# ktncktnc/diffusion-forcing-transformer

Measured on AMD Instinct MI355X. Metric: denoised latent frames/sec, DFoT RE10K 8f & 200f rollout @1/2/4/8 GPU, higher is better.
Workload: dtype bf16

## Files before the change

### diffusion-forcing-transformer_amd/capi.py

```python
from __future__ import annotations

import ctypes as C
import os

_HERE = os.path.dirname(os.path.abspath(__file__))
LIB_PATH = os.environ.get("DFOT_LIB", os.path.join(_HERE, "libdfot_hip.so"))

OK, ERR_ARG, ERR_SHAPE, ERR_HIP, ERR_STATE, ERR_NAME = range(6)


class DfotError(RuntimeError):
    def __init__(self, code: int, message: str):
        super().__init__(f"libdfot_hip error {code}: {message}")
        self.code = code


class UViTConfig(C.Structure):
    _fields_ = [
        ("channels", C.c_int32 * 4), ("emb_channels", C.c_int32), ("num_updown_blocks", C.c_int32 * 3),
        ("num_mid_blocks", C.c_int32), ("num_heads", C.c_int32), ("in_channels", C.c_int32),
        ("resolution", C.c_int32), ("max_tokens", C.c_int32), ("cond_dim", C.c_int32), ("noise_dim", C.c_int32),
        ("rope_theta", C.c_float), ("eps", C.c_float),
    ]

# ... 23 lines not shown
ATTN_MAP_OFF, ATTN_MAP_FRAME, ATTN_MAP_FULL = -1, 0, 1


_P, _I, _L, _F = C.c_void_p, C.c_int, C.c_int64, C.c_float
_I32 = C.c_int32


class GemmDesc(C.Structure):
    _fields_ = [
        ("amode", _I32), ("epi", _I32), ("variant", _I32),
        ("A", _P), ("lda", _L), ("W", _P), ("ldw", _L),
        ("M", _I32), ("N", _I32), ("K", _I32), ("H", _I32), ("Wd", _I32), ("Cin", _I32),
        ("live", _P), ("bias", _P), ("bias_rows", _I32),
        ("out_f32", _P), ("out_bf16", _P), ("ldo", _L),
        ("resid", _P), ("resid_bf", _P),
        ("gate", _P), ("gate_index", _P), ("ldg", _L), ("gate_rows", _I32),
        ("act", _I32), ("pre_act", _P), ("raw", _P), ("ldraw", _L), ("tr_rows", _I32),
        ("gn_part", _P), ("gn_rows_per_bt", _I32), ("gn_cpg", _I32),
        ("out2", _P), ("ldo2", _L), ("split", _I32),
        ("q", _P), ("k", _P), ("v", _P),
        ("qw", _P), ("kw", _P), ("rope_cs", _P),
        ("heads", _I32), ("d", _I32), ("ntok", _I32), ("qscale", _F), ("dstride", _I32), ("eps", _F),
        ("ksplit", _I32), ("slice_stride", _L),
    ]


SIGNATURES = {
    "dfot_last_error": (C.c_char_p, []),
    "dfot_version": (_I, []),
    "dfot_uvit_create": (_I, [C.POINTER(UViTConfig), C.POINTER(_P)]),
    "dfot_uvit_destroy": (_I, [_P]),
    "dfot_uvit_num_params": (_I, [_P]),
    "dfot_uvit_param_name": (C.c_char_p, [_P, _I]),
    "dfot_uvit_param_shape": (_I, [_P, _I, C.POINTER(_L), C.POINTER(_I)]),
    "dfot_uvit_load_weight": (_I, [_P, C.c_char_p, _P, C.POINTER(_L), _I, _P]),
    "dfot_uvit_finalize": (_I, [_P, _P]),
    "dfot_uvit_reserve": (_I, [_P, _I]),
    "dfot_uvit_workspace_bytes": (C.c_size_t, [_P]),
    "dfot_uvit_set_option": (_I, [_P, C.c_char_p, _I]),
    "dfot_uvit_query": (_I, [_P, C.c_char_p, C.POINTER(C.c_double)]),
    "dfot_uvit_attn_timing": (_I, [_P, C.POINTER(C.c_double), C.POINTER(_L)]),
    "dfot_uvit_forward": (_I, [_P, _P, _P, _P, _P, _P, _I, _P]),
    "dfot_uvit_set_conditions": (_I, [_P, _P, _P, _I, _P]),
    "dfot_uvit_forward_cached": (_I, [_P, _P, _P, _P, _I, _P]),
    "dfot_uvit_forward_cached_live": (_I, [_P, _P, _P, _P, _I, _P, _P]),
    "dfot_uvit_forward_cached_masks": (_I, [_P, _P, _P, _P, _I, _P, _P, _P]),
    "dfot_uvit_read_tap": (_I, [_P, C.c_char_p, _P, C.c_size_t, _P]),
    "dfot_uvit3d_create": (_I, [C.POINTER(UViT3DConfig), C.POINTER(_P)]),
    "dfot_uvit3d_config_bytes": (_L, []),
    "dfot_uvit3d_forward": (_I, [_P, _P, _P, _P, _P, _P, _I, _P]),
    "dfot_uvit3d_forward_live": (_I, [_P, _P, _P, _P, _P, _P, _I, _P, _P]),
    "dfot_op_gn_film_silu": (_I, [_P, _P, _P, _P, _P, _P, _P, _P, _I, _I, _I, _I, _P]),
    "dfot_op_rms_film": (_I, [_P, _P, _P, _P, _P, _P, _L, _I, _I, _I, _F, _P]),
    "dfot_dit_create": (_I, [C.POINTER(DiTConfig), C.POINTER(_P)]),
    "dfot_dit_create_f": (_I, [C.POINTER(DiTConfigF), C.POINTER(_P)]),
    "dfot_dit_destroy": (_I, [_P]),
    "dfot_dit_num_params": (_I, [_P]),
    "dfot_dit_param_name": (C.c_char_p, [_P, _I]),
    "dfot_dit_param_shape": (_I, [_P, _I, C.POINTER(_L), C.POINTER(_I)]),
    "dfot_dit_load_weight": (_I, [_P, C.c_char_p, _P, C.POINTER(_L), _I, _P]),
    "dfot_dit_finalize": (_I, [_P, _P]),
    "dfot_dit_reserve": (_I, [_P, _I]),
    "dfot_dit_workspace_bytes": (C.c_size_t, [_P]),
    "dfot_dit_set_option": (_I, [_P, C.c_char_p, _I]),
    "dfot_dit_attn_timing": (_I, [_P, C.POINTER(C.c_double), C.POINTER(_L)]),
    "dfot_dit_forward": (_I, [_P, _P, _P, _P, _I, _I, _P]),
    "dfot_dit_forward_cond": (_I, [_P, _P, _P, _P, _P, _P, _P, _I, _I, _P]),
    "dfot_dit_forward_f": (_I, [_P, _P, _P, _P, _P, _P, _P, _I, _I, _P]),
    "dfot_dit_read_tap": (_I, [_P, C.c_char_p, _P, C.c_size_t, _P]),
    "dfot_dit_capture_attention": (_I, [_P, C.POINTER(_I32), _I, _I, C.c_size_t]),
    "dfot_dit_attention_map_shape": (_I, [_P, _I, C.POINTER(_L), C.POINTER(_I)]),
    "dfot_dit_read_attention_map": (_I, [_P, _I, _P, C.c_size_t, _P]),
    "dfot_dit_train_create": (_I, [C.POINTER(DiTConfig), C.POINTER(_P)]),
    "dfot_dit_train_create_f": (_I, [C.POINTER(DiTConfigF), C.POINTER(_P)]),
    "dfot_facmat_train_create": (_I, [C.POINTER(DiTConfigF), C.POINTER(_P)]),
    "dfot_facdit_train_create": (_I, [C.POINTER(DiTConfigF), C.POINTER(_P)]),
    "dfot_dit_train_destroy": (_I, [_P]),
    "dfot_dit_train_num_params": (_I, [_P]),
    "dfot_dit_train_param_name": (C.c_char_p, [_P, _I]),
    "dfot_dit_train_param_shape": (_I, [_P, _I, C.POINTER(_L), C.POINTER(_I)]),
    "dfot_dit_train_param_offset": (_L, [_P, _I]),
    "dfot_dit_train_total_numel": (_L, [_P]),
    "dfot_dit_train_workspace_bytes": (C.c_size_t, [_P]),
    "dfot_dit_train_attach": (_I, [_P, _P, _P]),
    "dfot_dit_train_reserve": (_I, [_P, _I]),
    "dfot_dit_train_sync_weights": (_I, [_P, _P]),
    "dfot_dit_train_forward": (_I, [_P, _P, _P, _P, _I, _I, _P]),
    "dfot_dit_train_forward_cond": (_I, [_P, _P, _P, _P, _P, _P, _P, _I, _I, _P]),
    "dfot_dit_train_load_buffer": (_I, [_P, C.c_char_p, _P, _L, _P]),
    "dfot_dit_train_forward_f": (_I, [_P, _P, _P, _P, _P, _P, _P, _I, _I, _P]),
    "dfot_dit_train_input_grad": (_I, [_P, _P, _P]),
    "dfot_dit_train_backward": (_I, [_P, _P, _P]),
    "dfot_vloss_grad": (_I, [_P] * 7 + [_I, _I, _L, _I, _P]),
    "dfot_sumsq": (_I, [_P, _L, _P, _P]),
    "dfot_adamw_step": (_I, [_P, _P, _P, _P, _L, _F, _F, _F, _F, _F, _I, _P, _F, _P, _F, _P]),
    "dfot_ray_encode": (_I, [_P, _P, _I, _I, _I, _P]),
    "dfot_ray_encode_normalized": (_I, [_P, _P, _I, _I, _I, _P]),
    "dfot_hg_prepare": (_I, [_P, _P, _P, _P, _P, _I, _I, _I, _L, _P]),
    "dfot_ddim_compose": (_I, [_P] * 11 + [_I, _I, _I, _L, _P]),
    "dfot_ddim_compose_tokw": (_I, [_P] * 11 + [_I, _I, _I, _L, _P]),
    "dfot_ddim_noise": (_I, [_P] * 5 + [_I, _I, _I, _L, _I, _P]),
    "dfot_vpred_loss": (_I, [_P] * 9 + [_I, _I, _L, _P]),
    "dfot_vpred_loss_scratch_floats": (_L, [_I, _I, _L]),
    "dfot_vspace_loss": (_I, [_P] * 9 + [_I, _I, _L, _P]),
    "dfot_op_gemm": (_I, [_P, _I, _P, _P, _P, _I, _I, _I, _I, _P]),
    "dfot_op_conv3x3": (_I, [_P, _P, _P, _P, _I, _I, _I, _I, _I, _I, _P]),
# ... 133 lines not shown
```

### diffusion-forcing-transformer_amd/csrc/kernels.h

```cpp
#pragma once
#include "common.h"

namespace dfot {

int launch_noise_emb(const float* k, const float* freqs, const float* phases, const float* w1, const float* b1,
                     const float* w2, const float* b2, float* hidden, float* out, int bt, int ndim, int e, hipStream_t s);
int launch_uvit3d_emb(const float* k, const float* freqs, const float* phases, const float* w1, const float* b1, const float* w2,
                      const float* b2, const float* cond, const uint8_t* cond_mask, const float* a_w1, const float* a_b1,
                      const float* a_w2, const float* a_b2, float* out, int bt, int ndim, int cdim, int e, int tokens, hipStream_t s);
int launch_embed_input(const float* x, const float* w, const float* b, float* out, int bt, int res, int cin, int c0,
                       hipStream_t s);
int launch_cond_repack(const float* cond, bf16* a, int bt, int res, int cdim, int kpad, hipStream_t s);
int launch_emb_pyramid(const bf16* emb0, bf16* emb1, bf16* emb2, bf16* emb3, int bt, int r0, int e, hipStream_t s);
int launch_project_output(const float* x0, const float* w, const float* b, float* out, int bt, int res, int c0, int cout,
                          hipStream_t s, const uint8_t* live = nullptr);
int launch_gn_partial_f32(const float* x, float* partial, int bt, int pixels, int c, hipStream_t s);
int launch_gn_partial_bf16(const bf16* x, float* partial, int bt, int pixels, int c, hipStream_t s);
int launch_gn_finalize(const float* partial, float* stats, int bt, int nblk, int pixels, int c, float eps, hipStream_t s);
int gn_partial_blocks(int pixels);
int launch_gn_apply_silu(const float* x, const float* stats, const float* gamma, const float* beta, bf16* out, int bt,
                         int pixels, int c, hipStream_t s, const uint8_t* live = nullptr);
struct FilmChunk {
  const bf16* w;
  const float* b;
  long out_off;
  int rows;
};
int launch_film_vec(const FilmChunk* table, int chunks, const float* nemb, float* sv, int bt, int e, hipStream_t s);
int launch_gn_film_silu(const bf16* h, const float* stats, const float* gamma, const float* beta, const bf16* fcache,
                        const float* sv, const uint8_t* cond_mask, bf16* out, int bt, int pixels, int c, int tokens,
                        hipStream_t s, const uint8_t* live = nullptr);
struct RmsPending {
  void* x;
  const float* bias;
  const float* s0;
  const float* s1;
  const float* s2;
};
int launch_rms_film(const float* x, const float* w, const bf16* fcache, const float* sv, const uint8_t* cond_mask, bf16* out,
                    long m, int c, int rows_per_bt, int tokens, float eps, hipStream_t s, const RmsPending* pend = nullptr);
int launch_rms_film_bf16(const bf16* x, const float* w, const bf16* fcache, const float* sv, const uint8_t* cond_mask, bf16* out,
                         long m, int c, int rows_per_bt, int tokens, float eps, hipStream_t s, const RmsPending* pend = nullptr);

int launch_pool2_bf16(const float* x, bf16* out, int bt, int h, int w, int c, hipStream_t s);
int launch_pool2_bf16_bf16in(const bf16* x, bf16* out, int bt, int h, int w, int c, hipStream_t s);
int launch_sub_bf16_bf16in(const bf16* a, const float* b, bf16* out, long n, hipStream_t s, const uint8_t* live = nullptr, long frame_elems = 0);
int launch_upsample_add_bf16(const float* t, const bf16* skip, bf16* out, int bt, int h, int w, int c, hipStream_t s, const uint8_t* live = nullptr);
int launch_gn_apply_silu_bf16in(const bf16* x, const float* stats, const float* gamma, const float* beta, bf16* out, int bt, int pixels, int c,
                                hipStream_t s, const uint8_t* live = nullptr);
int launch_embed_input_bf16(const float* x, const float* w, const float* b, bf16* out, int bt, int res, int cin, int c0, hipStream_t s);
int launch_project_output_bf16(const bf16* x0, const float* w, const float* b, float* out, int bt, int res, int c0, int cout, hipStream_t s,
                               const uint8_t* live = nullptr);
int launch_sub_bf16(const float* a, const float* b, bf16* out, long n, hipStream_t s, const uint8_t* live = nullptr, long frame_elems = 0);
int launch_upsample_add(const float* t, const float* skip, float* out, int bt, int h, int w, int c, hipStream_t s, const uint8_t* live = nullptr);
int launch_ray_encode(const float* poses, float* out, int b, int t, int res, int normalized, hipStream_t s);
int launch_hg_prepare(const float* x, const float* noise, const float* qa, const float* qb, float* x_in, int batch,
                      int nfe, int tokens, long f, hipStream_t s);
int launch_ddim_compose(const float* x, const float* x_in, const float* v, const float* sa, const float* s1,
                        const float* an, const float* cn, const float* keep, const float* weight, const uint8_t* gen,
                        float* x_next, int batch, int nfe, int tokens, long f, bool weight_per_token, hipStream_t s);
int launch_ddim_noise(const float* noise, const float* sigma, const float* weight, const uint8_t* gen, float* x_next, int batch, int nfe,
                      int tokens, long f, bool weight_per_token, hipStream_t s);
int vloss_chunks(long f);
int launch_vloss(const float* x, const float* noise, const float* v, const float* a, const float* sg, const float* w,
                 float* x_pred, float* partial, float* loss, int batch, int tokens, long f, bool vspace, hipStream_t s);
int launch_wgrad_nt(const bf16* a, long lda, const bf16* b, long ldb, float* out, int m, int n, long rows, int slices, hipStream_t s, int img_h = 0,
                    int img_w = 0, int sdy = 0, int sdx = 0, int all_taps = 0);
struct WgradPlan {
  int form, slices;
};
WgradPlan wgrad_plan(int m, int n, long rows, long max_slices);
int launch_wgrad_conv_taps(const bf16* dy, const bf16* x, float* out, int co, int ci, long pix, int slices, int img_h, int img_w, hipStream_t s);
int wgrad_conv_tiles(int co, int ci, int* target);
int launch_wgrad_nt_plan(const bf16* a, long lda, const bf16* b, long ldb, float* out, int m, int n, long rows, WgradPlan plan, hipStream_t s);
int launch_vloss_grad(const float* x, const float* noise, const float* v, const float* a, const float* sg, const float* coef, float* dv,
                      int batch, int tokens, long f, bool vspace, hipStream_t s);
int launch_sumsq(const float* x, long n, float* out, hipStream_t s);
int launch_adamw(float* p, const float* g, float* m, float* v, long n, float lr, float b1, float b2, float eps, float wd, int step,
                 const float* sumsq, float max_norm, float* ema, float ema_decay, hipStream_t s);
int launch_f32_to_bf16(const float* src, bf16* dst, long n, hipStream_t s);
int launch_bf16_to_f32(const bf16* src, float* dst, long n, hipStream_t s);
int launch_equal_bits(const void* a, const void* b, long bytes, int* differs, hipStream_t s);
int launch_pack_rows(const float* src, bf16* dst, const int* map, int rows, int k, int kpad, long ldd, int col0,
                     hipStream_t s);
int launch_pack_conv3(const float* src, bf16* dst, int co, int ci, hipStream_t s);
int launch_gather_f32(const float* src, float* dst, const int* map, int n, hipStream_t s);
int launch_nhwc_to_nchw(const float* src, float* dst, int bt, int p, int c, hipStream_t s);
int launch_bf16_nhwc_to_nchw(const bf16* src, float* dst, int bt, int p, int c, hipStream_t s);

struct AttnScratch {
  float* p = nullptr;
  size_t bytes = 0;
};
// ... 46 lines not shown
```

### diffusion-forcing-transformer_amd/csrc/kernels.hip

```cpp
#include "kernels.h"
#include "dfot_hip.h"

namespace dfot {

typedef __attribute__((ext_vector_type(4))) float float4v;
typedef __attribute__((ext_vector_type(2))) float float2v;

__device__ __forceinline__ float wave_sum(float v) {
#pragma unroll
  for (int o = 32; o > 0; o >>= 1) v += __shfl_xor(v, o);
  return v;
}

template <bool FOURIER>
__global__ __launch_bounds__(256) void noise_mlp_kernel(const float* __restrict__ in, const float* __restrict__ freqs,
                                                        const float* __restrict__ phases, const float* __restrict__ w,
                                                        const float* __restrict__ b, float* __restrict__ out, int kdim,
                                                        int e) {
  const int lane = threadIdx.x & 63, wave = threadIdx.x >> 6;
  const int row = blockIdx.x * 4 + wave;
  const int bt = blockIdx.y;
  if (row >= e) return;
  float acc = 0.f;
  for (int i = lane; i < kdim; i += 64) {
    float f;
    if constexpr (FOURIER) {
      f = cosf(__fadd_rn(__fmul_rn(in[bt], freqs[i]), phases[i])) * 1.41421356237309515f;
    } else {
      f = in[(long)bt * kdim + i];
    }
    acc += w[(long)row * kdim + i] * f;
  }
  acc = wave_sum(acc);
  if (lane == 0) out[(long)bt * e + row] = FOURIER ? silu_f(acc + b[row]) : acc + b[row];
}

int launch_noise_emb(const float* k, const float* freqs, const float* phases, const float* w1, const float* b1,
                     const float* w2, const float* b2, float* hidden, float* out, int bt, int ndim, int e, hipStream_t s) {
  hipLaunchKernelGGL(noise_mlp_kernel<true>, dim3(cdiv(e, 4), bt), dim3(256), 0, s, k, freqs, phases, w1, b1, hidden, ndim, e);
  DFOT_CHECK_HIP(hipGetLastError());
  hipLaunchKernelGGL(noise_mlp_kernel<false>, dim3(cdiv(e, 4), bt), dim3(256), 0, s, hidden, nullptr, nullptr, w2, b2, out, e, e);
  DFOT_CHECK_HIP(hipGetLastError());
  return DFOT_OK;
}

constexpr int EMB_MAX = 1024;
constexpr int EMB_THREADS = 512;
__device__ __forceinline__ float emb_row_dot(const float* __restrict__ wrow, const float* in, int kdim, int lane) {
  float acc = 0.f;
  for (int i = lane; i < kdim; i += 64) acc += wrow[i] * in[i];
  return wave_sum(acc);
}
__global__ __launch_bounds__(EMB_THREADS) void uvit3d_emb_kernel(const float* __restrict__ k, const float* __restrict__ freqs,
                                                                 const float* __restrict__ phases, const float* __restrict__ w1,
// ... 766 lines not shown
  if (POSE && use_pose) {
#pragma unroll 4
    for (int it = 0; it < GN_ROWS_IT; ++it, pix += PPI) {
      const bf16x8 hv = *reinterpret_cast<const bf16x8*>(h + pix * C + c0);
      const bf16x8 fs = *reinterpret_cast<const bf16x8*>(fcache + pix * 2 * C + col);
      const bf16x8 fh = *reinterpret_cast<const bf16x8*>(fcache + pix * 2 * C + col + 32);
      bf16x8 o;
#pragma unroll
      for (int j = 0; j < 8; ++j) {
        const float sc = svs[j] + bf2f(fs[j]), sh = svh[j] + bf2f(fh[j]);
        o[j] = f2bf(silu_f(k.norm(bf2f(hv[j]), j) * (1.f + sc) + sh));
      }
      *reinterpret_cast<bf16x8*>(out + pix * C + c0) = o;
    }
  } else {
#pragma unroll 4
    for (int it = 0; it < GN_ROWS_IT; ++it, pix += PPI) {
      const bf16x8 hv = *reinterpret_cast<const bf16x8*>(h + pix * C + c0);
      bf16x8 o;
#pragma unroll
      for (int j = 0; j < 8; ++j) o[j] = f2bf(silu_f(k.norm(bf2f(hv[j]), j) * (1.f + svs[j]) + svh[j]));
      *reinterpret_cast<bf16x8*>(out + pix * C + c0) = o;
    }
  }
}

template <bool POSE>
static int launch_gn_film_silu_t(const bf16* h, const float* stats, const float* gamma, const float* beta, const bf16* fcache,
                                 const float* sv, const uint8_t* cond_mask, bf16* out, int bt, int pixels, int c, int tokens,
                                 hipStream_t s, const uint8_t* live) {
  if ((c == 128 || c == 256) && pixels % ((256 / (c / 8)) * GN_ROWS_IT) == 0) {
    const int grid = bt * (pixels / ((256 / (c / 8)) * GN_ROWS_IT));
    if (c == 128)
      hipLaunchKernelGGL((gn_film_silu_rows_kernel<128, POSE>), dim3(grid), dim3(256), 0, s, h, stats, gamma, beta, fcache, sv, cond_mask, out, pixels, tokens, live);
    else
      hipLaunchKernelGGL((gn_film_silu_rows_kernel<256, POSE>), dim3(grid), dim3(256), 0, s, h, stats, gamma, beta, fcache, sv, cond_mask, out, pixels, tokens, live);
    DFOT_CHECK_HIP(hipGetLastError());
    return DFOT_OK;
  }
  const long total8 = (long)bt * pixels * (c / 8);
  DFOT_REQUIRE(total8 < (1L << 31), DFOT_ERR_SHAPE, "groupnorm apply: %ld work items exceed the 32-bit index range", total8);
  hipLaunchKernelGGL(gn_film_silu_kernel<POSE>, dim3(cdiv(total8, 256)), dim3(256), 0, s, h, stats, gamma, beta, fcache, sv,
                     cond_mask, out, total8, pixels, c, tokens, live);
  DFOT_CHECK_HIP(hipGetLastError());
  return DFOT_OK;
}
int launch_gn_film_silu(const bf16* h, const float* stats, const float* gamma, const float* beta, const bf16* fcache,
                        const float* sv, const uint8_t* cond_mask, bf16* out, int bt, int pixels, int c, int tokens,
                        hipStream_t s, const uint8_t* live) {
  return fcache ? launch_gn_film_silu_t<true>(h, stats, gamma, beta, fcache, sv, cond_mask, out, bt, pixels, c, tokens, s, live)
                : launch_gn_film_silu_t<false>(h, stats, gamma, beta, nullptr, sv, nullptr, out, bt, pixels, c, tokens, s, live);
}

template <int MAXCH, bool PEND, typename TS, bool POSE>
__global__ __launch_bounds__(256) void rms_film_kernel(const TS* x, const float* __restrict__ w,
                                                       const bf16* __restrict__ fcache, const float* __restrict__ sv,
                                                       const uint8_t* __restrict__ cond_mask, bf16* __restrict__ out,
                                                       long m, int c, int rows_per_bt, int tokens, float eps, TS* xw,
                                                       const float* __restrict__ pbias, const float* __restrict__ p0,
                                                       const float* __restrict__ p1, const float* __restrict__ p2) {
  const long row = (long)blockIdx.x * 4 + (threadIdx.x >> 6);
  if (row >= m) return;
  const int lane = threadIdx.x & 63;
  const int nch = c / 8;
  const TS* src = x + row * c;
  float v[MAXCH][8];
  float ss = 0.f;
#pragma unroll
  for (int k = 0; k < MAXCH; ++k) {
    const int ch = lane + 64 * k;
    if (ch < nch) {
      stream_ld8(src + ch * 8, v[k]);
      if constexpr (PEND) {
        const long o = row * c + ch * 8;
#pragma unroll
        for (int hf = 0; hf < 2; ++hf) {
          float4v add = *reinterpret_cast<const float4v*>(pbias + ch * 8 + 4 * hf) + *reinterpret_cast<const float4v*>(p0 + o + 4 * hf) +
                        *reinterpret_cast<const float4v*>(p1 + o + 4 * hf);
          if (p2) add += *reinterpret_cast<const float4v*>(p2 + o + 4 * hf);
#pragma unroll
          for (int j = 0; j < 4; ++j) v[k][4 * hf + j] += add[j];
        }
        stream_st8(xw + o, v[k]);
        if constexpr (sizeof(TS) == 2) {
#pragma unroll
          for (int j = 0; j < 8; ++j) v[k][j] = bf2f(f2bf(v[k][j]));
        }
      }
#pragma unroll
      for (int j = 0; j < 8; ++j) ss += v[k][j] * v[k][j];
    }
  }
  ss = wave_sum(ss);
  const float rs = rsqrtf(ss / (float)c + eps);
  const int bt = (int)(row / rows_per_bt);
  bool use_pose = false;
  if constexpr (POSE) use_pose = !(cond_mask && cond_mask[(unsigned)bt / (unsigned)tokens]);
#pragma unroll
  for (int k = 0; k < MAXCH; ++k) {
    const int ch = lane + 64 * k;
    if (ch < nch) {
      const int c0 = ch * 8;
      const int col = (c0 >> 5) * 64 + (c0 & 31);
      const float* svp = sv + (long)bt * 2 * c + col;
      float sc[8], sh[8];
#pragma unroll
      for (int j = 0; j < 8; ++j) {
        sc[j] = svp[j];
        sh[j] = svp[32 + j];
      }
      if (POSE && use_pose) {
        const bf16x8 fs = *reinterpret_cast<const bf16x8*>(fcache + row * 2 * c + col);
        const bf16x8 fh = *reinterpret_cast<const bf16x8*>(fcache + row * 2 * c + col + 32);
#pragma unroll
        for (int j = 0; j < 8; ++j) {
          sc[j] += bf2f(fs[j]);
          sh[j] += bf2f(fh[j]);
        }
      }
      bf16x8 o;
#pragma unroll
      for (int j = 0; j < 8; ++j) o[j] = f2bf(v[k][j] * rs * w[c0 + j] * (1.f + sc[j]) + sh[j]);
      *reinterpret_cast<bf16x8*>(out + row * c + c0) = o;
    }
  }
}
template <typename TS, bool POSE>
static int launch_rms_film_p(const TS* x, const float* w, const bf16* fcache, const float* sv, const uint8_t* cond_mask, bf16* out,
                             long m, int c, int rows_per_bt, int tokens, float eps, hipStream_t s, const RmsPending* pend) {
  DFOT_REQUIRE(c % 8 == 0 && c <= 8 * 64 * 3, DFOT_ERR_SHAPE, "rms_film: channels %d unsupported", c);
#define RMS_CALL(MC, P)                                                                                                             \
  hipLaunchKernelGGL((rms_film_kernel<MC, P, TS, POSE>), dim3(cdiv(m, 4)), dim3(256), 0, s, x, w, fcache, sv, cond_mask, out, m, c, rows_per_bt, \
                     tokens, eps, P ? (TS*)pend->x : nullptr, P ? pend->bias : nullptr, P ? pend->s0 : nullptr, P ? pend->s1 : nullptr, P ? pend->s2 : nullptr)
  if (pend) {
    DFOT_REQUIRE(pend->x && pend->bias && pend->s0 && pend->s1, DFOT_ERR_ARG, "rms_film: pending sum needs a target, a bias and two slices");
    if (c <= 8 * 64 * 2) RMS_CALL(2, true); else RMS_CALL(3, true);
  } else {
    if (c <= 8 * 64 * 2) RMS_CALL(2, false); else RMS_CALL(3, false);
  }
#undef RMS_CALL
  DFOT_CHECK_HIP(hipGetLastError());
  return DFOT_OK;
}
template <typename TS>
static int launch_rms_film_t(const TS* x, const float* w, const bf16* fcache, const float* sv, const uint8_t* cond_mask, bf16* out,
                             long m, int c, int rows_per_bt, int tokens, float eps, hipStream_t s, const RmsPending* pend) {
  return fcache ? launch_rms_film_p<TS, true>(x, w, fcache, sv, cond_mask, out, m, c, rows_per_bt, tokens, eps, s, pend)
                : launch_rms_film_p<TS, false>(x, w, nullptr, sv, nullptr, out, m, c, rows_per_bt, tokens, eps, s, pend);
}
int launch_rms_film(const float* x, const float* w, const bf16* fcache, const float* sv, const uint8_t* cond_mask, bf16* out,
                    long m, int c, int rows_per_bt, int tokens, float eps, hipStream_t s, const RmsPending* pend) {
  return launch_rms_film_t<float>(x, w, fcache, sv, cond_mask, out, m, c, rows_per_bt, tokens, eps, s, pend);
}
int launch_rms_film_bf16(const bf16* x, const float* w, const bf16* fcache, const float* sv, const uint8_t* cond_mask, bf16* out,
                         long m, int c, int rows_per_bt, int tokens, float eps, hipStream_t s, const RmsPending* pend) {
  return launch_rms_film_t<bf16>(x, w, fcache, sv, cond_mask, out, m, c, rows_per_bt, tokens, eps, s, pend);
}

template <typename TIN>
__global__ void pool2_bf16_kernel(const TIN* __restrict__ x, bf16* __restrict__ out, long total4, int h, int w, int c) {
  const long idx = (long)blockIdx.x * blockDim.x + threadIdx.x;
  if (idx >= total4) return;
  const unsigned iu = (unsigned)idx, cq = (unsigned)(c / 4), w2 = (unsigned)(w / 2), h2 = (unsigned)(h / 2);
  const int c4 = (int)(iu % cq);
  const unsigned pix = iu / cq;
  const int ox = (int)(pix % w2), oy = (int)((pix / w2) % h2);
  const long bt = pix / (w2 * h2);
  const TIN* base = x + ((bt * h + 2 * oy) * w + 2 * ox) * (long)c + c4 * 4;
  const float4v a = stream_ld4(base);
  const float4v b = stream_ld4(base + c);
  const float4v cc = stream_ld4(base + (long)w * c);
  const float4v dd = stream_ld4(base + (long)w * c + c);
  bf16x4 o;
#pragma unroll
  for (int j = 0; j < 4; ++j) o[j] = f2bf((a[j] + b[j] + cc[j] + dd[j]) * 0.25f);
  *reinterpret_cast<bf16x4*>(out + pix * c + c4 * 4) = o;
}
int launch_pool2_bf16(const float* x, bf16* out, int bt, int h, int w, int c, hipStream_t s) {
  const long total4 = (long)bt * (h / 2) * (w / 2) * (c / 4);
  DFOT_REQUIRE(total4 < (1L << 31), DFOT_ERR_SHAPE, "pool2: %ld work items exceed the 32-bit index range", total4);
  hipLaunchKernelGGL(pool2_bf16_kernel<float>, dim3(cdiv(total4, 256)), dim3(256), 0, s, x, out, total4, h, w, c);
  DFOT_CHECK_HIP(hipGetLastError());
  return DFOT_OK;
}
int launch_pool2_bf16_bf16in(const bf16* x, bf16* out, int bt, int h, int w, int c, hipStream_t s) {
  const long total4 = (long)bt * (h / 2) * (w / 2) * (c / 4);
  DFOT_REQUIRE(total4 < (1L << 31), DFOT_ERR_SHAPE, "pool2: %ld work items exceed the 32-bit index range", total4);
  hipLaunchKernelGGL(pool2_bf16_kernel<bf16>, dim3(cdiv(total4, 256)), dim3(256), 0, s, x, out, total4, h, w, c);
  DFOT_CHECK_HIP(hipGetLastError());
  return DFOT_OK;
}

template <typename TIN, typename TB = TIN>
__global__ void sub_bf16_kernel(const TIN* __restrict__ a, const TB* __restrict__ b, bf16* __restrict__ out, long n4,
                                const uint8_t* __restrict__ live, long frame4) {
  const long idx = (long)blockIdx.x * blockDim.x + threadIdx.x;
  if (idx >= n4) return;
  if (live && !live[idx / frame4]) return;
  const float4v x = stream_ld4(a + idx * 4);
  const float4v y = stream_ld4(b + idx * 4);
  bf16x4 o;
#pragma unroll
  for (int j = 0; j < 4; ++j) o[j] = f2bf(x[j] - y[j]);
  *reinterpret_cast<bf16x4*>(out + idx * 4) = o;
}
int launch_sub_bf16(const float* a, const float* b, bf16* out, long n, hipStream_t s, const uint8_t* live, long frame_elems) {
  DFOT_REQUIRE(n % 4 == 0 && (!live || (frame_elems > 0 && frame_elems % 4 == 0)), DFOT_ERR_SHAPE, "sub: length %ld must be a multiple of 4", n);
  hipLaunchKernelGGL((sub_bf16_kernel<float, float>), dim3(cdiv(n / 4, 256)), dim3(256), 0, s, a, b, out, n / 4, live, live ? frame_elems / 4 : 1L);
  DFOT_CHECK_HIP(hipGetLastError());
// ... 525 lines not shown
```

### diffusion-forcing-transformer_amd/csrc/uvit.hip

```cpp
#include <algorithm>
#include <cmath>
#include <cstdarg>
#include <cstdlib>
#include <cstring>
#include <functional>
#include <map>
#include <string>
#include <vector>

#include "dfot_hip.h"
#include "gemm.h"
#include "kernels.h"

namespace dfot {

static thread_local char g_err[1024] = "";
void set_error(const char* fmt, ...) {
  va_list ap;
  va_start(ap, fmt);
  vsnprintf(g_err, sizeof(g_err), fmt, ap);
  va_end(ap);
}
const char* get_error() { return g_err; }

// ... 939 lines not shown
  h->last_batch = batch;
  return launch_project_output_bf16(h->XB[0], h->pout_w, h->pout_b, out, bt, c.resolution, h->ch[0], c.in_channels, s, live_frames);
}

extern "C" {

int dfot_uvit_forward(dfot_uvit_t h, const float* x, const float* noise_levels, const float* external_cond,
                      const uint8_t* external_cond_mask, float* out, int batch, void* stream) {
  DFOT_REQUIRE(h && x && noise_levels && out, DFOT_ERR_ARG, "forward: null argument");
  int rc = dfot_uvit_set_conditions(h, external_cond, external_cond_mask, batch, stream);
  if (rc) return rc;
  return dfot_uvit_forward_cached(h, x, noise_levels, out, batch, stream);
}

int dfot_uvit3d_forward_live(dfot_uvit_t h, const float* x, const float* noise_levels, const float* external_cond,
                             const uint8_t* external_cond_mask, float* out, int batch, const uint8_t* live_frames, void* stream) {
  DFOT_REQUIRE(h && x && noise_levels && out, DFOT_ERR_ARG, "uvit3d_forward: null argument");
  DFOT_REQUIRE(h->posefree, DFOT_ERR_STATE, "uvit3d_forward: the handle is a pose model (dfot_uvit_create); call dfot_uvit_forward");
  DFOT_REQUIRE(h->finalized, DFOT_ERR_STATE, "uvit3d_forward: weights not finalized");
  DFOT_REQUIRE(batch > 0 && batch <= h->max_batch, DFOT_ERR_STATE, "uvit3d_forward: batch %d exceeds reserved %d", batch, h->max_batch);
  DFOT_REQUIRE(!external_cond || h->act_dim > 0, DFOT_ERR_ARG,
               "uvit3d_forward: external_cond given, but the model was built with cond_dim 0 (no external_cond_embedding)");
  hipStream_t s = (hipStream_t)stream;
  const uint8_t* mask = (external_cond && h->act_dropout) ? external_cond_mask : nullptr;
  int rc = launch_uvit3d_emb(noise_levels, h->ne_freqs, h->ne_phases, h->ne_w1, h->ne_b1, h->ne_w2, h->ne_b2, external_cond, mask, h->ac_w1,
                             h->ac_b1, h->ac_w2, h->ac_b2, h->nemb, batch * h->T, h->cfg.noise_dim, h->act_dim, h->E, h->T, s);
  if (rc) return rc;
  h->have_mask = false;
  return forward_from_emb(h, x, out, batch, live_frames, nullptr, s);
}

int dfot_uvit3d_forward(dfot_uvit_t h, const float* x, const float* noise_levels, const float* external_cond,
                        const uint8_t* external_cond_mask, float* out, int batch, void* stream) {
  return dfot_uvit3d_forward_live(h, x, noise_levels, external_cond, external_cond_mask, out, batch, nullptr, stream);
}

int dfot_op_gn_film_silu(const void* h, const float* stats, const float* gamma, const float* beta, const void* fcache, const float* sv,
                         const uint8_t* cond_mask, void* out, int bt, int pixels, int c, int tokens, void* stream) {
  DFOT_REQUIRE(h && stats && gamma && beta && sv && out, DFOT_ERR_ARG, "op_gn_film_silu: null argument");
  DFOT_REQUIRE(bt > 0 && pixels > 0 && tokens > 0 && c > 0 && c % 32 == 0, DFOT_ERR_SHAPE,
               "op_gn_film_silu: bt %d, pixels %d, tokens %d must be positive and channels %d a multiple of 32", bt, pixels, tokens, c);
  return launch_gn_film_silu((const bf16*)h, stats, gamma, beta, (const bf16*)fcache, sv, cond_mask, (bf16*)out, bt, pixels, c, tokens,
                             (hipStream_t)stream);
}
int dfot_op_rms_film(const void* x, const float* w, const void* fcache, const float* sv, const uint8_t* cond_mask, void* out, int64_t m,
                     int c, int rows_per_bt, int tokens, float eps, void* stream) {
  DFOT_REQUIRE(x && w && sv && out, DFOT_ERR_ARG, "op_rms_film: null argument");
  DFOT_REQUIRE(m > 0 && rows_per_bt > 0 && tokens > 0 && c > 0 && c % 32 == 0 && m % rows_per_bt == 0, DFOT_ERR_SHAPE,
               "op_rms_film: rows %ld must be a positive multiple of rows_per_bt %d, channels %d a multiple of 32", (long)m, rows_per_bt, c);
  return launch_rms_film_bf16((const bf16*)x, w, (const bf16*)fcache, sv, cond_mask, (bf16*)out, (long)m, c, rows_per_bt, tokens, eps,
                              (hipStream_t)stream);
}

int dfot_uvit_read_tap(dfot_uvit_t h, const char* name, float* out, size_t capacity, void* stream) {
  DFOT_REQUIRE(h && name && out, DFOT_ERR_ARG, "read_tap: null argument");
  DFOT_REQUIRE(h->last_batch > 0, DFOT_ERR_STATE, "read_tap: no forward has run");
  hipStream_t s = (hipStream_t)stream;
  const int bt = h->last_batch * h->T;
  if (!strcmp(name, "nemb")) {
    const size_t need = (size_t)bt * h->E;
    DFOT_REQUIRE(capacity >= need, DFOT_ERR_SHAPE, "read_tap: need %zu floats, got %zu", need, capacity);
    return copy_f32(out, h->nemb, need, s);
  }
  DFOT_REQUIRE(!(h->posefree && !strcmp(name, "pose_emb0")), DFOT_ERR_NAME, "read_tap: a pose-free handle has no tap 'pose_emb0'");
  auto pixels = [&](int l) { return h->r[l] * h->r[l]; };
  struct Tap { const char* n; int lvl; int c; const float* f; const bf16* b; };
  const Tap taps[] = {
      {"pose_emb0", 0, h->E, nullptr, h->emb[0]}, {"down0", 1, h->ch[1], h->HSA[0], nullptr},
      {"down1", 2, h->ch[2], h->HSA[1], nullptr}, {"down2", 3, h->ch[3], h->HSA[2], nullptr},
      {"mid", 3, h->ch[3], nullptr, h->XB[3]}, {"up2", 2, h->ch[2], nullptr, h->XB[2]},
      {"up1", 1, h->ch[1], nullptr, h->XB[1]}, {"up0", 0, h->ch[0], nullptr, h->XB[0]},
  };
  for (const Tap& t : taps) {
    if (strcmp(t.n, name)) continue;
    const size_t need = (size_t)bt * pixels(t.lvl) * t.c;
    DFOT_REQUIRE(capacity >= need, DFOT_ERR_SHAPE, "read_tap: need %zu floats, got %zu", need, capacity);
    return t.f ? launch_nhwc_to_nchw(t.f, out, bt, pixels(t.lvl), t.c, s)
               : launch_bf16_nhwc_to_nchw(t.b, out, bt, pixels(t.lvl), t.c, s);
  }
  set_error("read_tap: unknown tap '%s'", name);
  return DFOT_ERR_NAME;
}

int dfot_ray_encode(const float* raw_poses, float* out, int batch, int tokens, int resolution, void* stream) {
  DFOT_REQUIRE(raw_poses && out && batch > 0 && tokens > 0 && resolution > 0, DFOT_ERR_ARG, "ray_encode: bad argument");
  return launch_ray_encode(raw_poses, out, batch, tokens, resolution, 0, (hipStream_t)stream);
}

int dfot_ray_encode_normalized(const float* poses, float* out, int batch, int tokens, int resolution, void* stream) {
  DFOT_REQUIRE(poses && out && batch > 0 && tokens > 0 && resolution > 0, DFOT_ERR_ARG, "ray_encode_normalized: bad argument");
  return launch_ray_encode(poses, out, batch, tokens, resolution, 1, (hipStream_t)stream);
}

int dfot_hg_prepare(const float* x, const float* noise, const float* qa, const float* qb, float* x_in, int batch, int nfe,
                    int tokens, int64_t frame_elems, void* stream) {
  DFOT_REQUIRE(x && qa && qb && x_in, DFOT_ERR_ARG, "hg_prepare: null argument");
  return launch_hg_prepare(x, noise, qa, qb, x_in, batch, nfe, tokens, (long)frame_elems, (hipStream_t)stream);
}

int dfot_ddim_compose(const float* x, const float* x_in, const float* v, const float* sa, const float* s1, const float* an,
                      const float* cn, const float* keep, const float* weight, const uint8_t* gen, float* x_next, int batch,
                      int nfe, int tokens, int64_t frame_elems, void* stream) {
  DFOT_REQUIRE(x && x_in && v && sa && s1 && an && cn && keep && weight && gen && x_next, DFOT_ERR_ARG, "ddim_compose: null argument");
  return launch_ddim_compose(x, x_in, v, sa, s1, an, cn, keep, weight, gen, x_next, batch, nfe, tokens, (long)frame_elems, false,
                             (hipStream_t)stream);
}
// ... 102 lines not shown
```

### include/dfot_hip.h

```cpp
#ifndef DFOT_HIP_H_
#define DFOT_HIP_H_

#include <stddef.h>
#include <stdint.h>

#ifdef __cplusplus
extern "C" {
#endif

enum {
  DFOT_OK = 0,
  DFOT_ERR_ARG = 1,
  DFOT_ERR_SHAPE = 2,
  DFOT_ERR_HIP = 3,
  DFOT_ERR_STATE = 4,
  DFOT_ERR_NAME = 5
};

typedef struct dfot_uvit_s* dfot_uvit_t;

typedef struct {
  int32_t channels[4];
  int32_t emb_channels;
  int32_t num_updown_blocks[3];
// ... 12 lines not shown
int dfot_version(void);

int dfot_uvit_create(const dfot_uvit_config* cfg, dfot_uvit_t* out);
int dfot_uvit_destroy(dfot_uvit_t h);
int dfot_uvit_num_params(dfot_uvit_t h);
const char* dfot_uvit_param_name(dfot_uvit_t h, int index);
int dfot_uvit_param_shape(dfot_uvit_t h, int index, int64_t shape[4], int* ndim);
int dfot_uvit_load_weight(dfot_uvit_t h, const char* name, const float* data, const int64_t* shape, int ndim,
                          void* stream);
int dfot_uvit_finalize(dfot_uvit_t h, void* stream);
int dfot_uvit_reserve(dfot_uvit_t h, int max_batch);
size_t dfot_uvit_workspace_bytes(dfot_uvit_t h);
int dfot_uvit_set_option(dfot_uvit_t h, const char* key, int value);
int dfot_uvit_query(dfot_uvit_t h, const char* key, double* value);
int dfot_uvit_attn_timing(dfot_uvit_t h, double* total_ms, int64_t* launches);

int dfot_uvit_forward(dfot_uvit_t h, const float* x, const float* noise_levels, const float* external_cond,
                      const uint8_t* external_cond_mask, float* out, int batch, void* stream);
int dfot_uvit_set_conditions(dfot_uvit_t h, const float* external_cond, const uint8_t* external_cond_mask, int batch,
                             void* stream);
int dfot_uvit_forward_cached(dfot_uvit_t h, const float* x, const float* noise_levels, float* out, int batch,
                             void* stream);
int dfot_uvit_forward_cached_live(dfot_uvit_t h, const float* x, const float* noise_levels, float* out, int batch,
                                  const uint8_t* live_frames, void* stream);
int dfot_uvit_forward_cached_masks(dfot_uvit_t h, const float* x, const float* noise_levels, float* out, int batch,
                                   const uint8_t* live_frames, const uint8_t* fresh_frames, void* stream);
int dfot_uvit_read_tap(dfot_uvit_t h, const char* name, float* out, size_t capacity_floats, void* stream);

typedef struct {
  int32_t channels[4];
  int32_t emb_channels;
  int32_t num_updown_blocks[3];
  int32_t num_mid_blocks;
  int32_t num_heads;
  int32_t in_channels;
  int32_t resolution;
  int32_t max_tokens;
  int32_t cond_dim;
  int32_t noise_dim;
  float rope_theta;
  float eps;
  int32_t cond_dropout;
} dfot_uvit3d_config;
int dfot_uvit3d_create(const dfot_uvit3d_config* cfg, dfot_uvit_t* out);
int64_t dfot_uvit3d_config_bytes(void);
int dfot_uvit3d_forward(dfot_uvit_t h, const float* x, const float* noise_levels, const float* external_cond,
                        const uint8_t* external_cond_mask, float* out, int batch, void* stream);
int dfot_uvit3d_forward_live(dfot_uvit_t h, const float* x, const float* noise_levels, const float* external_cond,
                             const uint8_t* external_cond_mask, float* out, int batch, const uint8_t* live_frames, void* stream);
int dfot_op_gn_film_silu(const void* h, const float* stats, const float* gamma, const float* beta, const void* fcache, const float* sv,
                         const uint8_t* cond_mask, void* out, int bt, int pixels, int c, int tokens, void* stream);
int dfot_op_rms_film(const void* x, const float* w, const void* fcache, const float* sv, const uint8_t* cond_mask, void* out, int64_t m,
                     int c, int rows_per_bt, int tokens, float eps, void* stream);

typedef struct dfot_dit_s* dfot_dit_t;

typedef struct {
  int32_t hidden_size;
  int32_t depth;
  int32_t num_heads;
  int32_t patch_size;
  int32_t in_channels;
  int32_t height;
  int32_t width;
  int32_t max_tokens;
  int32_t mlp_hidden;
  int32_t noise_dim;
  int32_t timesteps;
  float rope_theta;
  float eps;
  int32_t variant;
  int32_t embed_col_dim;
  int32_t num_col_heads;
  int32_t num_row_heads;
  int32_t temporal_mlp_hidden;
  int32_t use_bias;
  int32_t cond_type;
  int32_t cond_dim;
  int32_t num_classes;
  int32_t cond_dropout;
  int32_t use_temporal_rope;
} dfot_dit_config;
enum { DFOT_COND_NONE = 0, DFOT_COND_ACTION = 1, DFOT_COND_LABEL = 2 };

typedef struct {
  dfot_dit_config base;
  int32_t fourier_noise;
} dfot_dit_config_f;

int dfot_dit_create(const dfot_dit_config* cfg, dfot_dit_t* out);
int dfot_dit_create_f(const dfot_dit_config_f* cfg, dfot_dit_t* out);
int dfot_dit_destroy(dfot_dit_t h);
int dfot_dit_num_params(dfot_dit_t h);
const char* dfot_dit_param_name(dfot_dit_t h, int index);
int dfot_dit_param_shape(dfot_dit_t h, int index, int64_t shape[4], int* ndim);
int dfot_dit_load_weight(dfot_dit_t h, const char* name, const float* data, const int64_t* shape, int ndim, void* stream);
int dfot_dit_finalize(dfot_dit_t h, void* stream);
int dfot_dit_reserve(dfot_dit_t h, int max_batch);
size_t dfot_dit_workspace_bytes(dfot_dit_t h);
int dfot_dit_set_option(dfot_dit_t h, const char* key, int value);
int dfot_dit_attn_timing(dfot_dit_t h, double* total_ms, int64_t* launches);
int dfot_dit_forward(dfot_dit_t h, const float* x, const int32_t* noise_levels, float* out, int batch, int tokens,
                     void* stream);
int dfot_dit_forward_cond(dfot_dit_t h, const float* x, const int32_t* noise_levels, const float* cond, const int32_t* labels,
                          const uint8_t* cond_mask, float* out, int batch, int tokens, void* stream);
int dfot_dit_forward_f(dfot_dit_t h, const float* x, const float* noise_levels, const float* cond, const int32_t* labels,
// ... 215 lines not shown
```

Baseline: 10.79.

## Pipeline RMS-FiLM rows per wave with hoisted per-frame vectors and double-buffered loads

The RMS-norm FiLM kernel now gives each wave a run of 4 or 8 consecutive rows of one frame instead of a single row. The per-frame norm weight, FiLM scale/shift and pending bias are loaded once into registers, and row loads are double-buffered so the next row's reads overlap the current row's reduction. The pending-sum path is specialised for 2 or 3 slices, and the unused fp32-input variant is removed. New C API entry points expose the pending RMS-FiLM, bf16 embed-input and project-output ops, which adds register pressure and alignment requirements in exchange for fewer redundant loads and more memory-level parallelism.

Result: no change. 10.85 (median of 6 runs) (+0.5%).

```diff
diff --git a/diffusion-forcing-transformer_amd/capi.py b/diffusion-forcing-transformer_amd/capi.py
--- a/diffusion-forcing-transformer_amd/capi.py
+++ b/diffusion-forcing-transformer_amd/capi.py
@@ -99,6 +99,9 @@
     "dfot_uvit3d_forward_live": (_I, [_P, _P, _P, _P, _P, _P, _I, _P, _P]),
     "dfot_op_gn_film_silu": (_I, [_P, _P, _P, _P, _P, _P, _P, _P, _I, _I, _I, _I, _P]),
     "dfot_op_rms_film": (_I, [_P, _P, _P, _P, _P, _P, _L, _I, _I, _I, _F, _P]),
+    "dfot_op_rms_film_pending": (_I, [_P, _P, _P, _P, _P, _P, _L, _I, _I, _I, _F, _P, _P, _P, _P, _P, _P]),
+    "dfot_op_embed_input_bf16": (_I, [_P, _P, _P, _P, _I, _I, _I, _I, _P]),
+    "dfot_op_project_output_bf16": (_I, [_P, _P, _P, _P, _I, _I, _I, _I, _P, _P]),
     "dfot_dit_create": (_I, [C.POINTER(DiTConfig), C.POINTER(_P)]),
     "dfot_dit_create_f": (_I, [C.POINTER(DiTConfigF), C.POINTER(_P)]),
     "dfot_dit_destroy": (_I, [_P]),
diff --git a/diffusion-forcing-transformer_amd/csrc/kernels.h b/diffusion-forcing-transformer_amd/csrc/kernels.h
--- a/diffusion-forcing-transformer_amd/csrc/kernels.h
+++ b/diffusion-forcing-transformer_amd/csrc/kernels.h
@@ -37,8 +37,6 @@
   const float* s1;
   const float* s2;
 };
-int launch_rms_film(const float* x, const float* w, const bf16* fcache, const float* sv, const uint8_t* cond_mask, bf16* out,
-                    long m, int c, int rows_per_bt, int tokens, float eps, hipStream_t s, const RmsPending* pend = nullptr);
 int launch_rms_film_bf16(const bf16* x, const float* w, const bf16* fcache, const float* sv, const uint8_t* cond_mask, bf16* out,
                          long m, int c, int rows_per_bt, int tokens, float eps, hipStream_t s, const RmsPending* pend = nullptr);
 
diff --git a/diffusion-forcing-transformer_amd/csrc/kernels.hip b/diffusion-forcing-transformer_amd/csrc/kernels.hip
--- a/diffusion-forcing-transformer_amd/csrc/kernels.hip
+++ b/diffusion-forcing-transformer_amd/csrc/kernels.hip
@@ -1,5 +1,7 @@
 #include "kernels.h"
 #include "dfot_hip.h"
+
+#include <type_traits>
 
 namespace dfot {
 
@@ -872,109 +874,185 @@
                 : launch_gn_film_silu_t<false>(h, stats, gamma, beta, nullptr, sv, nullptr, out, bt, pixels, c, tokens, s, live);
 }
 
-template <int MAXCH, bool PEND, typename TS, bool POSE>
-__global__ __launch_bounds__(256) void rms_film_kernel(const TS* x, const float* __restrict__ w,
+struct StreamRaw8 {
+  bf16x8 a;
+  __device__ __forceinline__ void load(const bf16* p) { a = *reinterpret_cast<const bf16x8*>(p); }
+  __device__ __forceinline__ void get(float (&v)[8]) const {
+#pragma unroll
+    for (int j = 0; j < 8; ++j) v[j] = bf2f(a[j]);
+  }
+};
+template <int MAXCH, int PEND, bool POSE>
+struct RmsRowRegs {
+  StreamRaw8 x[MAXCH];
+  float4v p[PEND ? MAXCH : 1][PEND ? PEND : 1][2];
+  bf16x8 fs[POSE ? MAXCH : 1], fh[POSE ? MAXCH : 1];
+};
+template <int MAXCH, int PEND, int RUN, bool POSE>
+__global__ __launch_bounds__(256) void rms_film_kernel(const bf16* x, const float* __restrict__ w,
                                                        const bf16* __restrict__ fcache, const float* __restrict__ sv,
                                                        const uint8_t* __restrict__ cond_mask, bf16* __restrict__ out,
-                                                       long m, int c, int rows_per_bt, int tokens, float eps, TS* xw,
+                                                       int nbt, int c, int rows_per_bt, int runs_per_bt, int tokens, float eps, bf16* xw,
                                                        const float* __restrict__ pbias, const float* __restrict__ p0,
                                                        const float* __restrict__ p1, const float* __restrict__ p2) {
-  const long row = (long)blockIdx.x * 4 + (threadIdx.x >> 6);
-  if (row >= m) return;
+  const unsigned wid = blockIdx.x * 4u + (threadIdx.x >> 6);
+  const int bt = (int)(wid / (unsigned)runs_per_bt);
+  if (bt >= nbt) return;
+  const int r0 = (int)(wid % (unsigned)runs_per_bt) * RUN;
+  const int nr = rows_per_bt - r0 < RUN ? rows_per_bt - r0 : RUN;
+  const long row0 = (long)bt * rows_per_bt + r0;
   const int lane = threadIdx.x & 63;
   const int nch = c / 8;
-  const TS* src = x + row * c;
-  float v[MAXCH][8];
-  float ss = 0.f;
+  bool valid[MAXCH];
+  int c0[MAXCH], col[MAXCH];
 #pragma unroll
   for (int k = 0; k < MAXCH; ++k) {
     const int ch = lane + 64 * k;
-    if (ch < nch) {
-      stream_ld8(src + ch * 8, v[k]);
-      if constexpr (PEND) {
-        const long o = row * c + ch * 8;
-#pragma unroll
-        for (int hf = 0; hf < 2; ++hf) {
-          float4v add = *reinterpret_cast<const float4v*>(pbias + ch * 8 + 4 * hf) + *reinterpret_cast<const float4v*>(p0 + o + 4 * hf) +
-                        *reinterpret_cast<const float4v*>(p1 + o + 4 * hf);
-          if (p2) add += *reinterpret_cast<const float4v*>(p2 + o + 4 * hf);
-#pragma unroll
-          for (int j = 0; j < 4; ++j) v[k][4 * hf + j] += add[j];
+    valid[k] = ch < nch;
+    c0[k] = (valid[k] ? ch : nch - 1) * 8;
+    col[k] = (c0[k] >> 5) * 64 + (c0[k] & 31);
+  }
+  float4v wv[MAXCH][2], scv[MAXCH][2], shv[MAXCH][2], pb[PEND ? MAXCH : 1][2];
+#pragma unroll
+  for (int k = 0; k < MAXCH; ++k) {
+    const float* svp = sv + (long)bt * 2 * c + col[k];
+#pragma unroll
+    for (int hf = 0; hf < 2; ++hf) {
+      wv[k][hf] = *reinterpret_cast<const float4v*>(w + c0[k] + 4 * hf);
+      scv[k][hf] = *reinterpret_cast<const float4v*>(svp + 4 * hf);
+      shv[k][hf] = *reinterpret_cast<const float4v*>(svp + 32 + 4 * hf);
+      if constexpr (PEND != 0) pb[k][hf] = *reinterpret_cast<const float4v*>(pbias + c0[k] + 4 * hf);
+    }
+  }
+  typedef RmsRowRegs<MAXCH, PEND, POSE> Row;
+  auto pipeline = [&](auto full, auto pose) {
+    constexpr bool FULL = decltype(full)::value, USE_POSE = decltype(pose)::value;
+    auto request = [&](Row& r, int i) {
+      const long row = row0 + (FULL || i < nr ? i : nr - 1);
+#pragma unroll
+      for (int k = 0; k < MAXCH; ++k) {
+        const long o = row * c + c0[k];
+        r.x[k].load(x + o);
+        if constexpr (PEND != 0) {
+#pragma unroll
+          for (int hf = 0; hf < 2; ++hf) {
+            r.p[k][0][hf] = *reinterpret_cast<const float4v*>(p0 + o + 4 * hf);
+            r.p[k][1][hf] = *reinterpret_cast<const float4v*>(p1 + o + 4 * hf);
+            if constexpr (PEND == 3) r.p[k][2][hf] = *reinterpret_cast<const float4v*>(p2 + o + 4 * hf);
+          }
         }
-        stream_st8(xw + o, v[k]);
-        if constexpr (sizeof(TS) == 2) {
+        if constexpr (USE_POSE) {
+          r.fs[k] = *reinterpret_cast<const bf16x8*>(fcache + row * 2 * c + col[k]);
+          r.fh[k] = *reinterpret_cast<const bf16x8*>(fcache + row * 2 * c + col[k] + 32);
+        }
+      }
+    };
+    auto finish = [&](const Row& r, long row) {
+      float v[MAXCH][8];
+      float ss = 0.f;
+#pragma unroll
+      for (int k = 0; k < MAXCH; ++k) {
+        r.x[k].get(v[k]);
+        if constexpr (PEND != 0) {
+#pragma unroll
+          for (int hf = 0; hf < 2; ++hf) {
+            float4v add = pb[k][hf] + r.p[k][0][hf] + r.p[k][1][hf];
+            if constexpr (PEND == 3) add += r.p[k][2][hf];
+#pragma unroll
+            for (int j = 0; j < 4; ++j) v[k][4 * hf + j] += add[j];
+          }
+          if (valid[k]) stream_st8(xw + row * c + c0[k], v[k]);
 #pragma unroll
           for (int j = 0; j < 8; ++j) v[k][j] = bf2f(f2bf(v[k][j]));
         }
+#pragma unroll
+        for (int j = 0; j < 8; ++j) v[k][j] = valid[k] ? v[k][j] : 0.f;
+#pragma unroll
+        for (int j = 0; j < 8; ++j) ss += v[k][j] * v[k][j];
       }
-#pragma unroll
-      for (int j = 0; j < 8; ++j) ss += v[k][j] * v[k][j];
-    }
-  }
-  ss = wave_sum(ss);
-  const float rs = rsqrtf(ss / (float)c + eps);
-  const int bt = (int)(row / rows_per_bt);
+      ss = wave_sum(ss);
+      const float rs = rsqrtf(ss / (float)c + eps);
+#pragma unroll
+      for (int k = 0; k < MAXCH; ++k) {
+        float sc[8], sh[8];
+#pragma unroll
+        for (int j = 0; j < 8; ++j) {
+          sc[j] = scv[k][j >> 2][j & 3];
+          sh[j] = shv[k][j >> 2][j & 3];
+        }
+        if constexpr (USE_POSE) {
+#pragma unroll
+          for (int j = 0; j < 8; ++j) {
+            sc[j] += bf2f(r.fs[k][j]);
+            sh[j] += bf2f(r.fh[k][j]);
+          }
+        }
+        bf16x8 o;
+#pragma unroll
+        for (int j = 0; j < 8; ++j)
+          o[j] = f2bf(__fmaf_rn(__fmul_rn(__fmul_rn(v[k][j], rs), wv[k][j >> 2][j & 3]), __fadd_rn(1.f, sc[j]), sh[j]));
+        if (valid[k]) *reinterpret_cast<bf16x8*>(out + row * c + c0[k]) = o;
+      }
+    };
+    Row ra, rb;
+    request(ra, 0);
+#pragma unroll
+    for (int i = 0; i < RUN; i += 2) {
+      request(rb, i + 1);
+      if (FULL || i < nr) finish(ra, row0 + i);
+      if (i + 2 < RUN) request(ra, i + 2);
+      if (FULL || i + 1 < nr) finish(rb, row0 + i + 1);
+    }
+  };
   bool use_pose = false;
-  if constexpr (POSE) use_pose = !(cond_mask && cond_mask[(unsigned)bt / (unsigned)tokens]);
-#pragma unroll
-  for (int k = 0; k < MAXCH; ++k) {
-    const int ch = lane + 64 * k;
-    if (ch < nch) {
-      const int c0 = ch * 8;
-      const int col = (c0 >> 5) * 64 + (c0 & 31);
-      const float* svp = sv + (long)bt * 2 * c + col;
-      float sc[8], sh[8];
-#pragma unroll
-      for (int j = 0; j < 8; ++j) {
-        sc[j] = svp[j];
-        sh[j] = svp[32 + j];
-      }
-      if (POSE && use_pose) {
-        const bf16x8 fs = *reinterpret_cast<const bf16x8*>(fcache + row * 2 * c + col);
-        const bf16x8 fh = *reinterpret_cast<const bf16x8*>(fcache + row * 2 * c + col + 32);
-#pragma unroll
-        for (int j = 0; j < 8; ++j) {
-          sc[j] += bf2f(fs[j]);
-          sh[j] += bf2f(fh[j]);
-        }
-      }
-      bf16x8 o;
-#pragma unroll
-      for (int j = 0; j < 8; ++j) o[j] = f2bf(v[k][j] * rs * w[c0 + j] * (1.f + sc[j]) + sh[j]);
-      *reinterpret_cast<bf16x8*>(out + row * c + c0) = o;
-    }
-  }
-}
-template <typename TS, bool POSE>
-static int launch_rms_film_p(const TS* x, const float* w, const bf16* fcache, const float* sv, const uint8_t* cond_mask, bf16* out,
+  if constexpr (POSE) use_pose = __builtin_amdgcn_readfirstlane(!(cond_mask && cond_mask[(unsigned)bt / (unsigned)tokens]));
+  if (nr == RUN) {
+    if (POSE && use_pose) pipeline(std::true_type{}, std::integral_constant<bool, POSE>{});
+    else pipeline(std::true_type{}, std::false_type{});
+  } else {
+    if (POSE && use_pose) pipeline(std::false_type{}, std::integral_constant<bool, POSE>{});
+    else pipeline(std::false_type{}, std::false_type{});
+  }
+}
+template <bool POSE>
+static int launch_rms_film_p(const bf16* x, const float* w, const bf16* fcache, const float* sv, const uint8_t* cond_mask, bf16* out,
                              long m, int c, int rows_per_bt, int tokens, float eps, hipStream_t s, const RmsPending* pend) {
   DFOT_REQUIRE(c % 8 == 0 && c <= 8 * 64 * 3, DFOT_ERR_SHAPE, "rms_film: channels %d unsupported", c);
-#define RMS_CALL(MC, P)                                                                                                             \
-  hipLaunchKernelGGL((rms_film_kernel<MC, P, TS, POSE>), dim3(cdiv(m, 4)), dim3(256), 0, s, x, w, fcache, sv, cond_mask, out, m, c, rows_per_bt, \
-                     tokens, eps, P ? (TS*)pend->x : nullptr, P ? pend->bias : nullptr, P ? pend->s0 : nullptr, P ? pend->s1 : nullptr, P ? pend->s2 : nullptr)
+  DFOT_REQUIRE(rows_per_bt > 0 && m % rows_per_bt == 0, DFOT_ERR_SHAPE, "rms_film: rows %ld must be whole frames of %d rows", m, rows_per_bt);
+  DFOT_REQUIRE((((uintptr_t)w | (uintptr_t)sv | (uintptr_t)(pend ? pend->bias : nullptr)) & 15) == 0, DFOT_ERR_ARG,
+               "rms_film: the norm weight, the FiLM vectors and the pending bias must be 16-byte aligned");
+  const int nbt = (int)(m / rows_per_bt);
+  const int run = (long)nbt * cdiv(rows_per_bt, 4) > 2048 ? 8 : 4;
+  const int runs_per_bt = cdiv(rows_per_bt, run);
+  const long waves = (long)nbt * runs_per_bt;
+  DFOT_REQUIRE(waves < (1L << 31), DFOT_ERR_SHAPE, "rms_film: %ld row runs exceed the 32-bit index range", waves);
+#define RMS_CALL_R(MC, P, R)                                                                                                        \
+  hipLaunchKernelGGL((rms_film_kernel<MC, P, R, POSE>), dim3(cdiv(waves, 4)), dim3(256), 0, s, x, w, fcache, sv, cond_mask, out, nbt, c, rows_per_bt, \
+                     runs_per_bt, tokens, eps, P ? (bf16*)pend->x : nullptr, P ? pend->bias : nullptr, P ? pend->s0 : nullptr, P ? pend->s1 : nullptr, P == 3 ? pend->s2 : nullptr)
+#define RMS_CALL(MC, P)          \
+  do {                           \
+    if (run == 8) RMS_CALL_R(MC, P, 8); \
+    else RMS_CALL_R(MC, P, 4);   \
+  } while (0)
   if (pend) {
     DFOT_REQUIRE(pend->x && pend->bias && pend->s0 && pend->s1, DFOT_ERR_ARG, "rms_film: pending sum needs a target, a bias and two slices");
-    if (c <= 8 * 64 * 2) RMS_CALL(2, true); else RMS_CALL(3, true);
+    if (pend->s2) {
+      if (c <= 8 * 64 * 2) RMS_CALL(2, 3); else RMS_CALL(3, 3);
+    } else {
+      if (c <= 8 * 64 * 2) RMS_CALL(2, 2); else RMS_CALL(3, 2);
+    }
   } else {
-    if (c <= 8 * 64 * 2) RMS_CALL(2, false); else RMS_CALL(3, false);
+    if (c <= 8 * 64 * 2) RMS_CALL(2, 0); else RMS_CALL(3, 0);
   }
 #undef RMS_CALL
-  DFOT_CHECK_HIP(hipGetLastError());
-  return DFOT_OK;
-}
-template <typename TS>
-static int launch_rms_film_t(const TS* x, const float* w, const bf16* fcache, const float* sv, const uint8_t* cond_mask, bf16* out,
-                             long m, int c, int rows_per_bt, int tokens, float eps, hipStream_t s, const RmsPending* pend) {
-  return fcache ? launch_rms_film_p<TS, true>(x, w, fcache, sv, cond_mask, out, m, c, rows_per_bt, tokens, eps, s, pend)
-                : launch_rms_film_p<TS, false>(x, w, nullptr, sv, nullptr, out, m, c, rows_per_bt, tokens, eps, s, pend);
-}
-int launch_rms_film(const float* x, const float* w, const bf16* fcache, const float* sv, const uint8_t* cond_mask, bf16* out,
-                    long m, int c, int rows_per_bt, int tokens, float eps, hipStream_t s, const RmsPending* pend) {
-  return launch_rms_film_t<float>(x, w, fcache, sv, cond_mask, out, m, c, rows_per_bt, tokens, eps, s, pend);
+#undef RMS_CALL_R
+  DFOT_CHECK_HIP(hipGetLastError());
+  return DFOT_OK;
 }
 int launch_rms_film_bf16(const bf16* x, const float* w, const bf16* fcache, const float* sv, const uint8_t* cond_mask, bf16* out,
                          long m, int c, int rows_per_bt, int tokens, float eps, hipStream_t s, const RmsPending* pend) {
-  return launch_rms_film_t<bf16>(x, w, fcache, sv, cond_mask, out, m, c, rows_per_bt, tokens, eps, s, pend);
+  return fcache ? launch_rms_film_p<true>(x, w, fcache, sv, cond_mask, out, m, c, rows_per_bt, tokens, eps, s, pend)
+                : launch_rms_film_p<false>(x, w, nullptr, sv, nullptr, out, m, c, rows_per_bt, tokens, eps, s, pend);
 }
 
 template <typename TIN>
diff --git a/diffusion-forcing-transformer_amd/csrc/uvit.hip b/diffusion-forcing-transformer_amd/csrc/uvit.hip
--- a/diffusion-forcing-transformer_amd/csrc/uvit.hip
+++ b/diffusion-forcing-transformer_amd/csrc/uvit.hip
@@ -1015,6 +1015,28 @@
                               (hipStream_t)stream);
 }
 
+int dfot_op_rms_film_pending(const void* x, const float* w, const void* fcache, const float* sv, const uint8_t* cond_mask, void* out, int64_t m,
+                             int c, int rows_per_bt, int tokens, float eps, void* xw, const float* bias, const float* s0, const float* s1,
+                             const float* s2, void* stream) {
+  DFOT_REQUIRE(x && w && sv && out && xw && bias && s0 && s1, DFOT_ERR_ARG, "op_rms_film_pending: null argument");
+  DFOT_REQUIRE(m > 0 && rows_per_bt > 0 && tokens > 0 && c > 0 && c % 32 == 0 && m % rows_per_bt == 0, DFOT_ERR_SHAPE,
+               "op_rms_film_pending: rows %ld must be a positive multiple of rows_per_bt %d, channels %d a multiple of 32", (long)m, rows_per_bt, c);
+  const RmsPending pend{xw, bias, s0, s1, s2};
+  return launch_rms_film_bf16((const bf16*)x, w, (const bf16*)fcache, sv, cond_mask, (bf16*)out, (long)m, c, rows_per_bt, tokens, eps,
+                              (hipStream_t)stream, &pend);
+}
+int dfot_op_embed_input_bf16(const float* x, const float* w, const float* b, void* out, int bt, int res, int cin, int c0, void* stream) {
+  DFOT_REQUIRE(x && w && b && out, DFOT_ERR_ARG, "op_embed_input_bf16: null argument");
+  DFOT_REQUIRE(bt > 0 && res > 0 && cin > 0 && c0 > 0, DFOT_ERR_SHAPE, "op_embed_input_bf16: %d frames of %d -> %d channels at resolution %d", bt, cin, c0, res);
+  return launch_embed_input_bf16(x, w, b, (bf16*)out, bt, res, cin, c0, (hipStream_t)stream);
+}
+int dfot_op_project_output_bf16(const void* x0, const float* w, const float* b, float* out, int bt, int res, int c0, int cout,
+                                const uint8_t* live_frames, void* stream) {
+  DFOT_REQUIRE(x0 && w && b && out, DFOT_ERR_ARG, "op_project_output_bf16: null argument");
+  DFOT_REQUIRE(bt > 0 && res > 0 && res % 2 == 0, DFOT_ERR_SHAPE, "op_project_output_bf16: %d frames at resolution %d", bt, res);
+  return launch_project_output_bf16((const bf16*)x0, w, b, out, bt, res, c0, cout, (hipStream_t)stream, live_frames);
+}
+
 int dfot_uvit_read_tap(dfot_uvit_t h, const char* name, float* out, size_t capacity, void* stream) {
   DFOT_REQUIRE(h && name && out, DFOT_ERR_ARG, "read_tap: null argument");
   DFOT_REQUIRE(h->last_batch > 0, DFOT_ERR_STATE, "read_tap: no forward has run");
diff --git a/include/dfot_hip.h b/include/dfot_hip.h
--- a/include/dfot_hip.h
+++ b/include/dfot_hip.h
@@ -88,6 +88,12 @@
                          const uint8_t* cond_mask, void* out, int bt, int pixels, int c, int tokens, void* stream);
 int dfot_op_rms_film(const void* x, const float* w, const void* fcache, const float* sv, const uint8_t* cond_mask, void* out, int64_t m,
                      int c, int rows_per_bt, int tokens, float eps, void* stream);
+int dfot_op_rms_film_pending(const void* x, const float* w, const void* fcache, const float* sv, const uint8_t* cond_mask, void* out, int64_t m,
+                             int c, int rows_per_bt, int tokens, float eps, void* xw, const float* bias, const float* s0, const float* s1,
+                             const float* s2, void* stream);
+int dfot_op_embed_input_bf16(const float* x, const float* w, const float* b, void* out, int bt, int res, int cin, int c0, void* stream);
+int dfot_op_project_output_bf16(const void* x0, const float* w, const float* b, float* out, int bt, int res, int c0, int cout,
+                                const uint8_t* live_frames, void* stream);
 
 typedef struct dfot_dit_s* dfot_dit_t;
 
```
